# sony/DiffRoll

Hardware: AMD Instinct MI355X
Metric: piano-roll frames/sec (200-step sample) (higher is better)
Workload: dtype f32

## Files before the change

diffroll_amd/csrc/device_common.h:

```cpp
#pragma once
#include "kernels.h"

#include <algorithm>
#include <cstdio>
#include <cstdlib>
#include <type_traits>

namespace dr {

typedef float f32x16 __attribute__((ext_vector_type(16)));
typedef float f32x4 __attribute__((ext_vector_type(4)));
typedef unsigned u32x4 __attribute__((ext_vector_type(4)));

#define DR_DEVINL __device__ __forceinline__

#ifndef DR_FAULT
#define DR_FAULT 0
#endif

#ifdef DR_BOUNDS
static __device__ unsigned long long g_bounds[4];
DR_DEVINL void bounds_fail(unsigned code, long a, long b) {
    if (atomicCAS(&g_bounds[0], 0ull, (unsigned long long)code) == 0ull) { g_bounds[1] = (unsigned long long)a; g_bounds[2] = (unsigned long long)b; }
    atomicAdd(&g_bounds[3], 1ull);
// ... 5 lines not shown
#define DR_CHECK_LDS(p, lo, hi, code) do { const unsigned o_ = lds_off(p); if (o_ < (unsigned)(lo) || o_ + 16u > (unsigned)(hi)) bounds_fail((code), o_, (hi)); } while (0)
static unsigned long long g_host_violations = 0;
static void host_extent(const void* p, size_t bytes, const char* what, const char* kernel) {
    if (!p || !bytes) return;
    hipDeviceptr_t base = nullptr;
    size_t size = 0;
    if (hipMemGetAddressRange(&base, &size, (hipDeviceptr_t)p) != hipSuccess) { (void)hipGetLastError(); return; }
    if ((const char*)p < (const char*)base || (const char*)p + bytes > (const char*)base + size) {
        ++g_host_violations;
        fprintf(stderr, "[DR_BOUNDS] %s: %s needs %zu bytes at +%zd of a %zu-byte allocation\n", kernel, what, bytes,
                (ssize_t)((const char*)p - (const char*)base), size);
    }
}
static void check_gemm_extents(const GemmArgs& a, int epi, int prec, const char* kernel) {
    const size_t slab = prec ? 24576 : 16384;
    const int mts = a.mt0 + a.MT;
    host_extent(a.Wp, (size_t)mts * a.kchunks * a.taps * slab, "packed weights", kernel);
    host_extent(a.bias, (size_t)mts * 128 * 4, "bias", kernel);
    if (epi == EPI_GATE) host_extent(a.bias2, (size_t)mts * 128 * 4, "bias2", kernel);
    const long nbx = a.x_bmod ? (a.NB < a.x_bmod ? a.NB : a.x_bmod) : a.NB;
    if (!prec) host_extent(a.X, (size_t)((nbx - 1) * a.x_bs + (long)(a.x_planes - 1) * a.x_ps + (long)(a.T - 1) * a.x_fs + 4) * 4, "X", kernel);
    const long nby = a.NB + (a.dual > 0 ? a.dual : 0);
    const long planes = (a.y_rows + 3) / 4;
    if (!(a.out_s3 & 1)) host_extent(a.Y, (size_t)((nby - 1) * a.y_bs + (planes - 1) * a.y_ps + (long)(a.T - 1) * a.y_fs + 4) * 4, "Y", kernel);
    if (a.Y2 && !(a.out_s3 & 2)) host_extent(a.Y2, (size_t)((nby - 1) * a.y2_bs + (planes - 1) * a.y_ps + (long)(a.T - 1) * a.y_fs + 4) * 4, "Y2", kernel);
    const long c_hi = a.c_b0 + (a.n_cond > 1 ? a.n_cond - 1 : 0), c_last = (a.c_n > 0 && c_hi >= a.c_n) ? a.c_n - 1 : c_hi;
    if (epi == EPI_GATE && a.cond) host_extent(a.cond, (size_t)(c_last * a.c_bs + (long)mts * 128 * a.T) * 4, "conditioner", kernel);
    if (epi == EPI_GATE && a.cond2) host_extent(a.cond2, (size_t)mts * 128 * a.T * 4, "conditioner (shared)", kernel);
    if (epi == EPI_RES_SKIP && a.skip && mts * 128 > a.y_rows)
        host_extent(a.skip, (size_t)((long)(a.NB - 1) * a.s_bs + (long)(mts * 128 - a.y_rows) * a.T) * 4, "skip", kernel);
    if (a.ws) host_extent(a.ws, a.ws_floats * 4, "split-K workspace", kernel);
    if (a.ws_cnt) host_extent(a.ws_cnt, a.ws_cnt_n * 4, "split-K counters", kernel);
}
#define DR_BOUNDS_TU(tag)                                                                                       \
    hipError_t read_bounds_##tag(unsigned long long* out4) {                                                    \
        hipError_t e = hipMemcpyFromSymbol(out4, HIP_SYMBOL(g_bounds), 4 * sizeof(unsigned long long));         \
        if (e == hipSuccess && g_host_violations) { if (!out4[0]) out4[0] = 999; out4[3] += g_host_violations; } \
        return e;                                                                                               \
    }                                                                                                           \
    hipError_t reset_bounds_##tag() {                                                                           \
        unsigned long long z[4] = {0, 0, 0, 0};                                                                 \
        g_host_violations = 0;                                                                                  \
        return hipMemcpyToSymbol(HIP_SYMBOL(g_bounds), z, sizeof z);                                            \
    }
#define DR_CHECK_EXTENTS(a, epi, prec, kernel) check_gemm_extents((a), (epi), (prec), (kernel))
// ... 123 lines not shown
```

diffroll_amd/csrc/gemm.hip:

```cpp
#include "gemm_body.h"

namespace dr {

Tuning& tuning() { static Tuning t; return t; }
std::atomic<unsigned>& tuning_epoch() { static std::atomic<unsigned> n{0}; return n; }
PlanKnobs plan_knobs() {
    const Tuning& t = tuning();
    PlanKnobs k;
    k.tile = t.tile; k.pw = t.pw; k.pw_nw = t.pw_nw; k.pwk = t.pwk; k.ksplit_max = t.ksplit_max;
    k.ksplit_blocks = t.ksplit_blocks; k.stack3 = t.stack3; k.stack_fl = t.stack_fl;
    return k;
}

DR_BOUNDS_TU(gemm)
hipError_t read_bounds(unsigned long long* out4) {
    unsigned long long t[4];
    hipError_t e;
    out4[0] = out4[1] = out4[2] = out4[3] = 0;
    hipError_t (*readers[])(unsigned long long*) = {read_bounds_gemm, read_bounds_stack, read_bounds_tail};
    for (auto rd : readers) {
        if ((e = rd(t)) != hipSuccess) return e;
        if (!out4[0] && t[0]) { out4[0] = t[0]; out4[1] = t[1]; out4[2] = t[2]; }
        out4[3] += t[3];
    }
// ... 23 lines not shown
    }
    return o;
}

template <int NI, int KS, int EPI, int PREC, int FOLDP = (NI == 1)>
__global__ __launch_bounds__(512) void gemm_kernel(const GemmArgs a) {
    extern __shared__ __attribute__((aligned(16))) char smem[];
    const BlockTile bt = block_tile(a, a.ksplit);
    gemm_body<NI, KS, EPI, PREC, 0, FOLDP>(a, smem, bt.mt, bt.nt, bt.ks);
}

template <int NW>
__global__ __launch_bounds__(256) void pw_kernel(const GemmArgs a) {
    const int wave = __builtin_amdgcn_readfirstlane(threadIdx.x >> 6);
    const BlockTile bt = block_tile(a, 1);
    pw_body<NW, 0, 0>(a, bt.mt + a.mt0, bt.nt, wave);
}

template <int NW>
__global__ __launch_bounds__(256) void pwk_kernel(const GemmArgs a) {
    __shared__ float4 part[4][NW][4][64];
    const int wave = __builtin_amdgcn_readfirstlane(threadIdx.x >> 6);
    const int lane = threadIdx.x & 63;
    const int r = lane & 31, hi = lane >> 5;
    constexpr int BN = 32 * NW;
    const int RT = a.MT * 4;
    const int rt = blockIdx.x % RT + a.mt0 * 4, nt = blockIdx.x / RT;
    const int mt = rt >> 2, sr = rt & 3;
    const int tps = (a.T + BN - 1) / BN;
    const int b = nt / tps;
    const int t0 = (nt % tps) * BN;
    const int NS = a.kchunks, NSW = NS >> 2;
    const int s0 = wave * NSW;

    const __amdgpu_buffer_rsrc_t wr = __builtin_amdgcn_make_buffer_rsrc(
        (void*)(a.Wp + (long)mt * NS * 4096), 0, (unsigned)NS * 16384u, 0x00020000);
    const __amdgpu_buffer_rsrc_t xr = __builtin_amdgcn_make_buffer_rsrc(
        (void*)(a.X + (long)b * a.x_bs), 0, (unsigned)(a.x_planes * a.x_ps * 4), 0x00020000);
    const int wvo = (hi * 128 + sr * 32 + r) * 16;
    const int xps = (int)a.x_ps * 4;
    int xvo[NW];
#pragma unroll
    for (int ni = 0; ni < NW; ++ni) xvo[ni] = hi * xps + min(t0 + ni * 32 + r, a.T - 1) * 16;
    struct BF { float4 v[4][NW]; };
    auto load_a = [&](int slab) { return load_a4(wr, wvo, slab, NS, 140); };
    auto load_b = [&](int slab) -> BF {
        BF o;
#pragma unroll
        for (int g = 0; g < 4; ++g)
#pragma unroll
            for (int ni = 0; ni < NW; ++ni)
                o.v[g][ni] = buffer_load_f4(xr, xvo[ni], (slab * 8 + g * 2) * xps);
        return o;
    };
    const int p0 = mt * 128 + sr * 32 + 8 * wave + 4 * hi;
    const bool res_rows = p0 < a.y_rows;
    const float4 ebias = *reinterpret_cast<const float4*>(a.bias + p0);
    const float4 ed2 = *reinterpret_cast<const float4*>(a.d2 + (a.tsel ? (long)a.tsel[b] * a.d2_ts : 0) + min(p0, a.y_rows - 4));
    float4 eop[NW];
    {
        const float* base = res_rows ? a.Y + (long)b * a.y_bs + (long)(p0 >> 2) * a.y_ps
                                     : a.skip + (long)b * a.s_bs + (long)((p0 - a.y_rows) >> 2) * a.T * 4;
        const long fs = res_rows ? a.y_fs : 4;
#pragma unroll
        for (int ni = 0; ni < NW; ++ni) eop[ni] = *reinterpret_cast<const float4*>(base + (long)min(t0 + ni * 32 + r, a.T - 1) * fs);
    }

    f32x16 acc[NW];
#pragma unroll
    for (int ni = 0; ni < NW; ++ni)
#pragma unroll
        for (int e = 0; e < 16; ++e) acc[ni][e] = 0.f;
    AF4 aA = load_a(s0), aB;
    BF bA = load_b(s0), bB;
    auto mma = [&](const AF4& af, const BF& bf) {
#pragma unroll
        for (int g = 0; g < 4; ++g) {
// ... 34 lines not shown
            f4arr(part[w][ni][wave][lane], u);
#pragma unroll
            for (int e = 0; e < 4; ++e) v[e] += u[e];
        }
        if (res_rows) {
            float* dst = a.Y + (long)b * a.y_bs + (long)(p0 >> 2) * a.y_ps + (long)t * a.y_fs;
            residual_quad(v, ebias, eop[ni], o);
            *reinterpret_cast<float4*>(dst) = make_float4(o[0], o[1], o[2], o[3]);
            if (a.Y2) {
                float o2[4];
                hd_quad(o, ed2, o2);
                float* dst2 = a.Y2 + (long)b * a.y2_bs + (long)(p0 >> 2) * a.y_ps + (long)t * a.y_fs;
                *reinterpret_cast<float4*>(dst2) = make_float4(o2[0], o2[1], o2[2], o2[3]);
            }
        } else {
            float* dst = a.skip + (long)b * a.s_bs + ((long)((p0 - a.y_rows) >> 2) * a.T + t) * 4;
            skip_quad(v, ebias, eop[ni], a.skip_init, o);
            *reinterpret_cast<float4*>(dst) = make_float4(o[0], o[1], o[2], o[3]);
        }
    }
}

template <int NW>
static hipError_t launch_pwk_t(const GemmArgs& a, hipStream_t s) {
    const int BN = 32 * NW;
    const int NT = a.NB * ((a.T + BN - 1) / BN);
    DR_CHECK_EXTENTS(a, EPI_RES_SKIP, 0, "pwk_kernel");
    hipLaunchKernelGGL((pwk_kernel<NW>), dim3((unsigned)(a.MT * 4 * NT)), dim3(256), 0, s, a);
    return hipGetLastError();
}
hipError_t launch_pointwise_ksplit(const GemmArgs& a, int NW, hipStream_t s) {
// ... 179 lines not shown
```

diffroll_amd/csrc/gemm_body.h:

```cpp
#pragma once
#include "device_common.h"

namespace dr {

DR_DEVINL void residual_quad(const float (&v)[4], const float4 bias, const float4 prev, float (&o)[4]) {
    float bb[4], pv[4];
    f4arr(bias, bb); f4arr(prev, pv);
#pragma unroll
    for (int e = 0; e < 4; ++e) o[e] = div_sqrt2(pv[e] + (v[e] + bb[e]));
}
DR_DEVINL void skip_quad(const float (&v)[4], const float4 bias, const float4 prev, const bool skip_init, float (&o)[4]) {
    float bb[4], pv[4];
    f4arr(bias, bb); f4arr(prev, pv);
#pragma unroll
    for (int e = 0; e < 4; ++e) o[e] = skip_init ? v[e] + bb[e] : (v[e] + bb[e]) + pv[e];
}
DR_DEVINL long cond_row(const GemmArgs& a, const int b) {
    int r = a.c_b0 + b;
    if (a.c_n > 0 && r >= a.c_n) r %= a.c_n;
    return r;
}
DR_DEVINL void gate_quad(const float (&v0)[4], const float (&v1)[4], const float4 bias0, const float4 bias1,
                         const float4 cond0, const float4 cond1, const bool has_c, float (&o)[4]) {
    float b0[4], b1[4], c0[4], c1[4];
// ... 69 lines not shown
                const int sg = pl / 6, rem = pl - sg * 6, pce = rem >> 1, kq = rem & 1;
                const int pc = min(chunk * (4 * KS) + sg * 2 + kq, last_plane);
                src = Xg + (long)pce * a.x_piece + (long)pc * a.x_ps;
            } else {
                src = Xg + (long)min(chunk * XP + pl, last_plane) * a.x_ps;
            }
            const __amdgpu_buffer_rsrc_t rsrc = __builtin_amdgcn_make_buffer_rsrc((void*)src, 0, recs, 0x00020000);
            const int voff = (t0 - halo + f) * (int)a.x_fs * 4;
            float4* dst = Xs + (((chunk - c0) & 1) * XP + pl) * FW + seg * 64;
            if (f < FW) DR_CHECK_LDS(dst + lane, lds_off(Xs), lds_off(Xs) + 2u * XP * FW * 16u, code_x);
            if (f < FW) __builtin_amdgcn_raw_ptr_buffer_load_lds(rsrc, (lds_ptr)dst, 16, voff, 0, 0, AUX);
        }
    };
    if constexpr (RBN != 0) {
        auto plane_of = [&](int pl) -> const float* {
            const int row0 = mt * 128 + pl * 4;
            return (row0 < a.y_rows) ? a.Y + (long)b * a.y_bs + (long)(row0 >> 2) * a.y_ps
                                     : a.skip + (long)b * a.s_bs + (long)((row0 - a.y_rows) >> 2) * a.T * 4;
        };
        dma_tile<RBN, AUX>(Rs, plane_of, a.T, t0, pw, 4, lane, code_r);
    }
    issue(c0);
    for (int chunk = c0; chunk < c1; ++chunk) {
#if DR_FAULT != 1
        asm volatile("s_waitcnt vmcnt(0)" ::: "memory");
        __syncthreads();
#else
        __builtin_amdgcn_s_barrier();
#endif
        if (chunk + 1 < c1) issue(chunk + 1);
    }
}

// ... 318 lines not shown
    for (int pass = 0; pass < npass; ++pass) {
        const int be = b + pass * a.dual;
        const float* cbase = nullptr;
        if constexpr (EPI == EPI_GATE)
            cbase = (be < a.n_cond || !a.cond2) ? a.cond + (be < a.n_cond ? cond_row(a, be) : 0L) * a.c_bs : a.cond2;
        float4 ebias[4];
        float4 ed2[4];
        {
            const float* bsrc = a.bias;
            if constexpr (EPI == EPI_GATE) bsrc = (be < a.n_cond) ? a.bias : a.bias2;
    #pragma unroll
            for (int q = 0; q < 4; ++q) ebias[q] = *reinterpret_cast<const float4*>(bsrc + mt * 128 + wave * 32 + 8 * q + 4 * hi);
            if constexpr (EPI == EPI_RELU || EPI == EPI_RES_SKIP) {
    #pragma unroll
                for (int q = 0; q < 4; ++q) {
                    const int p0 = min(mt * 128 + wave * 32 + 8 * q + 4 * hi, a.y_rows - 4);
                    ed2[q] = *reinterpret_cast<const float4*>(a.d2 + (a.tsel ? (long)a.tsel[be] * a.d2_ts : 0) + p0);
                }
            }
        }
    #pragma unroll
        for (int ni = 0; ni < NW; ++ni) {
            const int t = t0 + ni * 32 + r;
            if constexpr (EPI == EPI_RES_SKIP) {
    #pragma unroll
                for (int q = 0; q < 4; ++q) {
                    DR_CHECK_LDS(Rs + (wave * 8 + 2 * q + hi) * BN + ni * 32 + r, xs1, rs1, 110);
                    eop[ni][q] = Rs[(wave * 8 + 2 * q + hi) * BN + ni * 32 + r];
                }
            }
            if constexpr (EPI == EPI_GATE) {
// ... 22 lines not shown
    #pragma unroll
                        for (int e = 0; e < 4; ++e) o[e] = v0[e] * v0[e] + v1[e] * v1[e];
                    }
                    if (a.out_s3 & 1) {
                        store_s3_quad<COH>(a.Y + (long)be * a.y_bs, o, c0, t, a.T, a.y_rows >> 3, a.wt_store);
                    } else {
                        float* dst = a.Y + (long)be * a.y_bs + (long)(c0 >> 2) * a.y_ps + (long)t * a.y_fs;
                        store_f4<COH>(dst, make_float4(o[0], o[1], o[2], o[3]), a.wt_store);
                    }
                } else {
                    const int p0 = mt * 128 + wave * 32 + rq;
                    float v[4], o[4];
    #pragma unroll
                    for (int e = 0; e < 4; ++e) v[e] = acc[ni][4 * q + e];
                    if constexpr (EPI == EPI_RES_SKIP) {
                        if (p0 < a.y_rows) {
                            float* dst = a.Y + (long)be * a.y_bs + (long)(p0 >> 2) * a.y_ps + (long)t * a.y_fs;
                            residual_quad(v, ebias[q], eop[ni][q], o);
                            *reinterpret_cast<float4*>(dst) = make_float4(o[0], o[1], o[2], o[3]);
                            if (a.Y2) store_y2<COH, 0>(a, be, o, ed2[q], p0, t);
                        } else {
                            float* dst = a.skip + (long)be * a.s_bs + ((long)((p0 - a.y_rows) >> 2) * a.T + t) * 4;
                            skip_quad(v, ebias[q], eop[ni][q], a.skip_init, o);
                            *reinterpret_cast<float4*>(dst) = make_float4(o[0], o[1], o[2], o[3]);
                        }
                    } else {
                        if (p0 >= a.y_rows) continue;
                        float bb[4];
                        f4arr(ebias[q], bb);
    #pragma unroll
                        for (int e = 0; e < 4; ++e) {
                            if constexpr (EPI == EPI_PLAIN) o[e] = a.alpha * v[e] + bb[e];
                            else if constexpr (EPI == EPI_RELU) o[e] = fmaxf(a.alpha * v[e] + bb[e], 0.f);
                            else if constexpr (EPI == EPI_SILU) { const float z = v[e] + bb[e]; o[e] = z * sigmoidf_(z); }
                            else o[e] = logf(v[e] + 1e-6f);
                        }
                        float* dst = a.Y + (long)be * a.y_bs + (long)(p0 >> 2) * a.y_ps + (long)t * a.y_fs;
// ... 9 lines not shown
    if (a.dbg && blockIdx.x == 0 && tid == 0) {
        a.dbg[0] = tick1 - tick0;
        a.dbg[1] = clock64() - tick0;
    }
}

template <int NW, int COH, int RLDS, int TBN = 32 * NW, int EPI = EPI_RES_SKIP>
DR_DEVINL void pw_body(const GemmArgs& a, const int mt, const int nt, const int wave, float4* Rs = nullptr, const int foff = 0) {
    static_assert(EPI == EPI_RES_SKIP || EPI == EPI_RELU || EPI == EPI_PLAIN, "pw_body epilogues");
    static_assert(EPI == EPI_RES_SKIP || !RLDS, "the LDS-resident tile belongs to the residual / skip epilogue");
    constexpr int BN = TBN;
    int lane = threadIdx.x & 63;
    if constexpr (COH) asm volatile("" : "+v"(lane));
    const int r = lane & 31, hi = lane >> 5;
    const long long tick0 = a.dbg ? clock64() : 0;

    const int tps = (a.T + BN - 1) / BN;
    const int b = nt / tps;
    const int t0 = (nt % tps) * BN + foff;
    const int NS = a.kchunks;

    const __amdgpu_buffer_rsrc_t wr = __builtin_amdgcn_make_buffer_rsrc(
        (void*)(a.Wp + (long)mt * NS * 4096), 0, (unsigned)NS * 16384u, 0x00020000);
    const __amdgpu_buffer_rsrc_t xr = __builtin_amdgcn_make_buffer_rsrc(
        (void*)(a.X + (long)b * a.x_bs), 0, (unsigned)(a.x_planes * a.x_ps * 4), 0x00020000);
    const int wvo = (hi * 128 + wave * 32 + r) * 16;
    const int xps = (int)a.x_ps * 4;
    int xvo[NW];
#pragma unroll
    for (int ni = 0; ni < NW; ++ni) xvo[ni] = hi * xps + min(t0 + ni * 32 + r, a.T - 1) * 16;
// ... 28 lines not shown
            const float4 af = kB ? aB.v[g] : aA.v[g];
#pragma unroll
            for (int ni = 0; ni < NW; ++ni) acc[ni] = __builtin_amdgcn_mfma_f32_32x32x2f32(af.x, (kB ? bB.v[g][ni] : bA.v[g][ni]).x, acc[ni], 0, 0, 0);
#pragma unroll
            for (int ni = 0; ni < NW; ++ni) acc[ni] = __builtin_amdgcn_mfma_f32_32x32x2f32(af.y, (kB ? bB.v[g][ni] : bA.v[g][ni]).y, acc[ni], 0, 0, 0);
#pragma unroll
            for (int ni = 0; ni < NW; ++ni) acc[ni] = __builtin_amdgcn_mfma_f32_32x32x2f32(af.z, (kB ? bB.v[g][ni] : bA.v[g][ni]).z, acc[ni], 0, 0, 0);
#pragma unroll
            for (int ni = 0; ni < NW; ++ni) acc[ni] = __builtin_amdgcn_mfma_f32_32x32x2f32(af.w, (kB ? bB.v[g][ni] : bA.v[g][ni]).w, acc[ni], 0, 0, 0);
        }
        constexpr int NLD = 4 + 4 * NW, PER = (16 * NW) / NLD;
        sgb_spread<NLD, PER>();
        sgb<0x8, 16 * NW - NLD * PER>();
    };
    const int rowb = mt * 128 + wave * 32 + 4 * hi;
    const bool res_rows = rowb < a.y_rows;
    float4 ebias[4], ed2[4], eop[RLDS ? 1 : NW][4];
    auto load_epilogue = [&]() {
#pragma unroll
        for (int q = 0; q < 4; ++q) {
            ebias[q] = *reinterpret_cast<const float4*>(a.bias + rowb + 8 * q);
            if constexpr (EPI == EPI_RES_SKIP)
                ed2[q] = *reinterpret_cast<const float4*>(a.d2 + (a.tsel ? (long)a.tsel[b] * a.d2_ts : 0) + min(rowb + 8 * q, a.y_rows - 4));
        }
        if constexpr (RLDS || EPI != EPI_RES_SKIP) return;
        const float* base = res_rows ? a.Y + (long)b * a.y_bs + (long)(rowb >> 2) * a.y_ps
                                     : a.skip + (long)b * a.s_bs + (long)((rowb - a.y_rows) >> 2) * a.T * 4;
        const long qs = res_rows ? 2 * a.y_ps : (long)2 * a.T * 4;
        const long fs = res_rows ? a.y_fs : 4;
#pragma unroll
        for (int ni = 0; ni < NW; ++ni) {
            const int tc = min(t0 + ni * 32 + r, a.T - 1);
#pragma unroll
            for (int q = 0; q < 4; ++q) eop[ni][q] = *reinterpret_cast<const float4*>(base + q * qs + tc * fs);
        }
    };
    int slab = 0;
    const int pre = max(NS - 2, 0) & ~1;
    for (; slab < pre; slab += 2) {
        step(std::false_type{}, slab);
        step(std::true_type{}, slab + 1);
        if (a.dbg && slab == 0 && blockIdx.x == 0 && threadIdx.x == 0) a.dbg[2] = clock64() - tick0;
// ... 3 lines not shown
    __builtin_amdgcn_sched_barrier(0);
    for (; slab + 2 <= NS; slab += 2) {
        step(std::false_type{}, slab);
        step(std::true_type{}, slab + 1);
    }
    if (slab < NS) step(std::false_type{}, slab);
    const long long tick1 = a.dbg ? clock64() : 0;
    if constexpr (RLDS) load_epilogue();

#pragma unroll
    for (int ni = 0; ni < NW; ++ni) {
        const int t = t0 + ni * 32 + r;
        if (t >= a.T) continue;
#pragma unroll
        for (int q = 0; q < 4; ++q) {
            const int p0 = rowb + 8 * q;
            float v[4], o[4];
#pragma unroll
            for (int e = 0; e < 4; ++e) v[e] = acc[ni][4 * q + e];
            if constexpr (EPI != EPI_RES_SKIP) {
                if (p0 >= a.y_rows) continue;
                float bb[4];
                f4arr(ebias[q], bb);
#pragma unroll
                for (int e = 0; e < 4; ++e) {
                    o[e] = a.alpha * v[e] + bb[e];
                    if constexpr (EPI == EPI_RELU) o[e] = fmaxf(o[e], 0.f);
                }
                float* dst = a.Y + (long)b * a.y_bs + (long)(p0 >> 2) * a.y_ps + (long)t * a.y_fs;
                store_f4<COH>(dst, make_float4(o[0], o[1], o[2], o[3]), a.wt_store);
                continue;
// ... 1 lines not shown
            float4* rs = nullptr;
            if constexpr (RLDS) rs = Rs + (wave * 8 + 2 * q + hi) * BN + foff + ni * 32 + r;
#ifdef DR_BOUNDS
            if constexpr (RLDS) DR_CHECK_LDS(rs, lds_off(Rs), lds_off(Rs) + 32u * BN * 16u, 121);
#endif
            float4 pv;
            if constexpr (RLDS) pv = *rs;
            else pv = eop[ni][q];
            if (res_rows) {
                float* dst = a.Y + (long)b * a.y_bs + (long)(p0 >> 2) * a.y_ps + (long)t * a.y_fs;
                residual_quad(v, ebias[q], pv, o);
                if constexpr (RLDS) *rs = make_float4(o[0], o[1], o[2], o[3]);
                else *reinterpret_cast<float4*>(dst) = make_float4(o[0], o[1], o[2], o[3]);
                if (a.Y2) store_y2<0, COH>(a, b, o, ed2[q], p0, t);
            } else {
                float* dst = a.skip + (long)b * a.s_bs + ((long)((p0 - a.y_rows) >> 2) * a.T + t) * 4;
                skip_quad(v, ebias[q], pv, a.skip_init, o);
                if constexpr (RLDS) *rs = make_float4(o[0], o[1], o[2], o[3]);
                else *reinterpret_cast<float4*>(dst) = make_float4(o[0], o[1], o[2], o[3]);
            }
        }
    }
    if (a.dbg && blockIdx.x == 0 && threadIdx.x == 0) {
        a.dbg[0] = tick1 - tick0;
        a.dbg[1] = clock64() - tick0;
    }
}

template <int NJ, int KS, int EPI>
DR_DEVINL void gemm16_body(const GemmArgs& a, char* smem, const int mt, const int nt) {
    static_assert(EPI == EPI_GATE || EPI == EPI_RES_SKIP, "16x16 variant: hot kernels only");
// ... 111 lines not shown
        }
    }

    const int rowb = mt * 128 + wave * 32 + kq * 4;
    float4 ebias[RT], ed2[RT];
    const float* cbase = nullptr;
    if constexpr (EPI == EPI_GATE)
        cbase = (b < a.n_cond || !a.cond2) ? a.cond + (b < a.n_cond ? cond_row(a, b) : 0L) * a.c_bs : a.cond2;
    {
        const float* bsrc = a.bias;
        if constexpr (EPI == EPI_GATE) bsrc = (b < a.n_cond) ? a.bias : a.bias2;
#pragma unroll
        for (int rt = 0; rt < RT; ++rt) {
            ebias[rt] = *reinterpret_cast<const float4*>(bsrc + rowb + rt * 16);
            if constexpr (EPI == EPI_RES_SKIP)
                ed2[rt] = *reinterpret_cast<const float4*>(a.d2 + (a.tsel ? (long)a.tsel[b] * a.d2_ts : 0) + min(rowb + rt * 16, a.y_rows - 4));
        }
    }
#pragma unroll
    for (int ct = 0; ct < CT; ++ct) {
        const int t = t0 + ct * 16 + li;
        if constexpr (EPI == EPI_GATE) {
            float4 cnd[RT];
            const int tc = min(t, a.T - 1);
            const float* cb = cbase + (long)tc * 4;
#pragma unroll
            for (int rt = 0; rt < RT; ++rt) cnd[rt] = *reinterpret_cast<const float4*>(cb + (long)((rowb + rt * 16) >> 2) * a.T * 4);
            if (t >= a.T) continue;
            const bool has_c = b < a.n_cond || a.cond2 != nullptr;
            {
                const int c0 = mt * 64 + wave * 16 + kq * 4;
// ... 6 lines not shown
                } else {
                    float* dst = a.Y + (long)b * a.y_bs + (long)(c0 >> 2) * a.y_ps + (long)t * a.y_fs;
                    *reinterpret_cast<float4*>(dst) = make_float4(o[0], o[1], o[2], o[3]);
                }
            }
        } else {
            float4 pv4[RT];
#pragma unroll
            for (int rt = 0; rt < RT; ++rt) {
                DR_CHECK_LDS(Rs + ((wave * 32 + rt * 16) / 4 + kq) * BN + ct * 16 + li, xs1, rs1, 145);
                pv4[rt] = Rs[((wave * 32 + rt * 16) / 4 + kq) * BN + ct * 16 + li];
            }
            if (t >= a.T) continue;
#pragma unroll
            for (int rt = 0; rt < RT; ++rt) {
                const int p0 = rowb + rt * 16;
                float v[4], o[4];
                f4arr(acc[rt][ct], v);
                if (p0 < a.y_rows) {
                    float* dst = a.Y + (long)b * a.y_bs + (long)(p0 >> 2) * a.y_ps + (long)t * a.y_fs;
                    residual_quad(v, ebias[rt], pv4[rt], o);
                    *reinterpret_cast<float4*>(dst) = make_float4(o[0], o[1], o[2], o[3]);
                    if (a.Y2) store_y2<0, 0>(a, b, o, ed2[rt], p0, t);
                } else {
                    float* dst = a.skip + (long)b * a.s_bs + ((long)((p0 - a.y_rows) >> 2) * a.T + t) * 4;
                    skip_quad(v, ebias[rt], pv4[rt], a.skip_init, o);
                    *reinterpret_cast<float4*>(dst) = make_float4(o[0], o[1], o[2], o[3]);
                }
            }
        }
    }
}

}
```

diffroll_amd/csrc/kernels.h:

```cpp
#pragma once
#include <hip/hip_runtime.h>
#include <stdint.h>

#include <atomic>

#include "launch_plan.h"

namespace dr {


struct Tuning {
    std::atomic<int> pack_threads{16};
    std::atomic<int> tile{0};
    std::atomic<int> pw{1};
    std::atomic<int> pw_nw{0};
    std::atomic<int> pwk{1};
    std::atomic<int> ksplit_max{16};
    std::atomic<long> ksplit_blocks{0};
    std::atomic<int> one_ks{0};
    std::atomic<int> stack3{1};
    std::atomic<int> stack_fl{0};
    std::atomic<int> tail_t4{0};
    std::atomic<int> xcd_n{-1};
    std::atomic<int> xcd_model{1};
// ... 5 lines not shown
PlanKnobs plan_knobs();

struct GemmArgs {
    const float* Wp;
    const float* bias;
    const float* bias2;
    const float* X;
    long x_bs, x_ps, x_fs;
    long x_piece;
    int x_planes;
    int x_bmod;
    int NB, T;
    int taps, dil;
    int kchunks;
    int MT;
    int mt0;
    float* Y;
    long y_bs, y_ps, y_fs;
    long y2_bs;
    int out_s3;
    float* Y2;
    const float* d2;
    const int* tsel;
    long d2_ts;
    int y_rows;
    const float* cond;
    long c_bs;
    int c_b0, c_n;
    const float* cond2;
    int n_cond;
    int dual;
    float* skip;
    long s_bs;
    int skip_init;
    float alpha;
    int xcd_n;
    float* ws;
    unsigned* ws_cnt;
    size_t ws_floats, ws_cnt_n;
    int ksplit;
    long long* dbg;
    int lds_bytes;
    int fold128;
    int nofold64;
    int wt_store;
};

hipError_t init_kernels();
hipError_t read_bounds(unsigned long long* out4);
// ... 128 lines not shown
```

diffroll_amd/csrc/launch_plan.h:

```cpp
#pragma once
#include <algorithm>
#include <cstddef>

#include "../../include/diffroll_amd.h"

namespace dr {

enum Epilogue : int {
    EPI_PLAIN = 0,
    EPI_RELU = 1,
    EPI_SILU = 2,
    EPI_GATE = 3,
    EPI_RES_SKIP = 4,
    EPI_POWER = 5,
    EPI_LOG = 6
};

constexpr int DR_STACK_MAX_LAYERS = 30;
constexpr int STACK_GROUPS = 512;
constexpr size_t SK_WS_FLOATS = (size_t)16 << 20, SK_CNT_N = 4096;

struct PlanKnobs {
    int tile = 0, pw = 1, pw_nw = 0, pwk = 1, ksplit_max = 16;
    long ksplit_blocks = 0;
    int stack3 = 1, stack_fl = 0;
};

inline int gemm_block_frames(int NI) { return (NI == 3 || NI == 5) ? 32 * NI : 64 * NI; }
inline size_t gemm_lds_bytes(int NI, int KS, int taps, int dil, int prec, int epi) {
    const int halo = ((taps - 1) / 2) * dil;
    const int BN = gemm_block_frames(NI);
// ... 194 lines not shown
```

diffroll_amd/csrc/pack.hip:

```cpp
#include "engine_state.h"

#include <mutex>

namespace drh {

template <class F>
int parallel_for(dr_engine* e, int n, F fn) {
    const int cap = tuning().pack_threads;
    const int hw = (int)std::thread::hardware_concurrency();
    const int nt = std::max(1, std::min(std::min(n, cap), hw > 0 ? hw : 1));
    std::atomic<bool> failed{false};
    auto guarded = [&](int i) {
        try { fn(i); } catch (...) { failed.store(true); }
    };
    if (nt == 1) {
        for (int i = 0; i < n && !failed.load(); ++i) guarded(i);
    } else {
        std::atomic<int> next{0};
        std::vector<std::thread> th;
        try {
            for (int t = 0; t < nt; ++t)
                th.emplace_back([&]() { for (int i = next.fetch_add(1); i < n && !failed.load(); i = next.fetch_add(1)) guarded(i); });
        } catch (...) { failed.store(true); }
        for (auto& t : th) t.join();
// ... 174 lines not shown

int ensure_s3(dr_engine* e) {
    if (e->s3_ready || !e->committed) return DR_OK;
    const int C = e->C, Cp = e->Cp, L = e->L, K = e->K;
    std::vector<std::vector<uint16_t>> c3(L), o3(L);
    int prc = parallel_for(e, L, [&](int l) {
        const std::string pre = "residual_layers." + std::to_string(l) + ".";
        const auto& Wd = *find_param(e, pre + "dilated_conv.weight");
        const auto& Wo = *find_param(e, pre + "output_projection.weight");
        const int MTc = Cp / 64;
        c3[l] = pack_weights_s3(MTc, Cp / 32, K, [&](int pr, int ch, int j) {
            int mi, c; paired_row(pr, mi, c);
            return (c < C && ch < C) ? Wd[((size_t)(mi * C + c) * C + ch) * K + j] : 0.f;
        });
        o3[l] = pack_weights_s3(MTc, Cp / 32, 1, [&](int pr, int ch, int) {
            const int half = pr >= Cp, c = pr - half * Cp;
            return (c < C && ch < C) ? Wo[(size_t)(half * C + c) * C + ch] : 0.f;
        });
    });
    if (prc) return prc;
    for (int l = 0; l < L; ++l) {
        int rc;
        if ((rc = upload_bytes(e, c3[l].data(), c3[l].size() * 2, &e->layers[l].conv_w3)) ||
            (rc = upload_bytes(e, o3[l].data(), o3[l].size() * 2, &e->layers[l].out_w3)))
            return rc;
        c3[l] = {}; o3[l] = {};
    }
    { StagerLock sl; HIPCHK(e, sl.s->drain()); }
    e->s3_ready = true;
    return DR_OK;
}
// ... 56 lines not shown
        });
        k.bconv.assign(MTc * 128, 0.f); k.bconv_u.assign(MTc * 128, 0.f); k.bconv_z.assign(MTc * 128, 0.f); k.bcond.assign(MTc * 128, 0.f);
        for (int pr = 0; pr < MTc * 128; ++pr) {
            int mi, c; paired_row(pr, mi, c);
            if (c >= C) continue;
            const int o = mi * C + c;
            double sw = 0.0;
            for (int m = 0; m < NM; ++m) sw += (double)Wc[(size_t)o * NM + m];
            const float cu = (float)((double)Bc[o] - sw);
            k.bconv[pr] = Bd[o];
            k.bconv_u[pr] = Bd[o] + cu;
            k.bconv_z[pr] = Bd[o] + Bc[o];
            k.bcond[pr] = Bc[o];
        }
        k.pout = pack_weights(MTc, Cp / 32, 1, [&](int pr, int ch, int) {
            const int half = pr >= Cp, c = pr - half * Cp;
            return (c < C && ch < C) ? Wo[(size_t)(half * C + c) * C + ch] : 0.f;
        });
        k.bout.assign(MTc * 128, 0.f);
        for (int pr = 0; pr < 2 * Cp; ++pr) {
            const int half = pr >= Cp, c = pr - half * Cp;
            if (c < C) k.bout[pr] = Bo[half * C + c];
        }
    });
    if (rc) return rc;
    e->t_pack_s = now_s() - tp0;
    const double tu0 = now_s();
    for (int l = 0; l < L; ++l) {
        LayerW& lw = e->layers[l];
        lw.dil = 1;
        for (int q = 0; q < l % e->cfg.dilation_bound; ++q) lw.dil *= e->cfg.dilation_base;
        LayerPack& k = packs[l];
        if ((rc = upload(e, k.pconv, &lw.conv_w)) || (rc = upload(e, k.bconv, &lw.conv_b)) ||
            (rc = upload(e, k.bconv_u, &lw.conv_b_u)) || (rc = upload(e, k.bconv_z, &lw.conv_b_z)) ||
            (rc = upload(e, k.pcond, &lw.cond_w)) ||
            (rc = upload(e, k.bcond, &lw.cond_b)) || (rc = upload(e, k.pout, &lw.out_w)) ||
// ... 140 lines not shown
```

diffroll_amd/csrc/plan.hip:

```cpp
#include "engine_state.h"

namespace drh {

hipError_t launch_tiled(const GemmArgs& a, int epi, Tile t, hipStream_t s, int prec) {
    if (t.flavor == 3) return launch_pointwise_ksplit(a, t.n, s);
    if (t.flavor == 2) return launch_pointwise(a, t.n, s);
    return t.flavor == 1 ? launch_gemm16(a, epi, t.n, s) : launch_gemm(a, epi, t.n, s, prec);
}
void allow_splitk(const dr_engine* e, GemmArgs& a) {
    a.ws = e->sk_ws; a.ws_cnt = e->sk_cnt;
    a.ws_floats = SK_WS_FLOATS; a.ws_cnt_n = SK_CNT_N;
}

const float* g_zero_vecs[MAX_DEVICES] = {};
const float* zero_vec() {
    int dev = 0;
    (void)hipGetDevice(&dev);
    return (dev >= 0 && dev < MAX_DEVICES) ? g_zero_vecs[dev] : nullptr;
}

GemmArgs p4_gemm(const float* Wp, const float* bias, int MT, const float* X, int planes, int NB, int T) {
    GemmArgs a{};
    a.d2 = zero_vec();
    a.Wp = Wp; a.bias = bias ? bias : zero_vec(); a.MT = MT;
// ... 193 lines not shown
    const long act_bs = (long)Cp * T;
    const LayerW& w = e->layers[l];
    GemmArgs a = p4_gemm(prec ? w.out_w3 : w.out_w, w.out_b, Cp / 64, e->g, Cp / 4, NB, T);
    if (prec) s3_in(a, e->g3, Cp, T);
    p4_out(a, e->h, Cp / 4, T, Cp);
    if (l + 1 < L) {
        a.d2 = e->d_dtab + ((v.tsel ? 0 : (size_t)v.t * L) + l + 1) * Cp;
        a.tsel = v.tsel; a.d2_ts = (long)L * Cp;
        if (prec) { a.Y2 = e->hd3; a.y2_bs = act_bs + act_bs / 2; a.out_s3 = 2; }
        else { a.Y2 = e->hd; a.y2_bs = act_bs; }
    }
    a.skip = e->skip; a.s_bs = (long)Cp * T; a.skip_init = (l == 0);
    allow_splitk(e, a);
    if (e->stack_dbg_on && l + 2 == L) a.dbg = e->stack_dbg + 96;
    Tile tile = pick_pointwise_tile(k, Cp / 64, NB, T, prec);
    if (l + 1 == L && tile.flavor >= 2) {
        const int first = Cp / 128, count = Cp / 64 - first;
        const Tile half = pick_pointwise_tile(k, count, NB, T, prec, Cp / 32);
        if (half.flavor == tile.flavor) { tile = half; a.MT = count; a.mt0 = first; }
    }
    HIPCHK(e, launch_tiled(a, EPI_RES_SKIP, tile, v.st, prec));
    return DR_OK;
}

static int launch_tail_step(const Eval& v, const NetPlan& p, const PlanKnobs& k, TailPlan* tail) {
    dr_engine* e = v.e;
    const int Cp = e->Cp, L = e->L, T = v.T;
    NetPlan np{};
    bool prime = false;
    if (tail->next_t >= 0) {
        np = plan_network(NetShape{tail->next.NB, tail->next.n_cond, v.bmod, T, Cp, L, e->K, e->max_dil, e->prec, e->n_cus,
                                   e->fused.active(), e->opt_blocked, e->opt_tail, false, true}, k);
        prime = np.use_tail;
    }
    TailArgs ta{};
// ... 157 lines not shown
```

diffroll_amd/csrc/stack.hip:

```cpp
#include "gemm_body.h"
#include "persistent.h"

namespace dr {

DR_BOUNDS_TU(stack)

template <int FL, int FOLDP = 1, int PREC = 0>
__global__ __launch_bounds__(512) void stack_kernel(const StackArgs s_by_value) {
    extern __shared__ __attribute__((aligned(16))) char smem[];
    (void)s_by_value;
    typedef const __attribute__((address_space(4))) StackArgs* KernArgs;
    const KernArgs sp = (KernArgs)__builtin_amdgcn_kernarg_segment_ptr();
    const __attribute__((address_space(4))) StackArgs& s = *sp;
    static_assert(FL == 1 || FL == 2 || (FL == 5 && FOLDP == 1 && PREC == 0), "block flavours");
    constexpr int BN = FL == 5 ? 160 : 64 * FL;
    constexpr int RP = 32;
    constexpr int RWL = (BN + 63) / 64;
    const int wave = __builtin_amdgcn_readfirstlane(threadIdx.x >> 6);
    const int MT = s.Cp >> 6;
    const int MB = MT;
    const int tps = (s.T + BN - 1) / BN;
    const unsigned gsize = (unsigned)(MB * tps);
    int mt, nt, grp, member;
    if (s.xcd_n) {
// ... 4 lines not shown
        member = blockIdx.x % (int)gsize;
        grp = blockIdx.x / (int)gsize;
    }
    if (grp >= s.NB) return;
    mt = member % MB;
    nt = grp * tps + member / MB;
    const unsigned pending_timeout = __hip_atomic_load(s.derr, __ATOMIC_RELAXED, __HIP_MEMORY_SCOPE_AGENT);
    DR_CHECK(grp >= 0 && grp < 512 && (long)grp * gsize + member < 1024, 130, grp, member);
    unsigned* ctr = s.bar + 4 * grp;
    const long act_bs = (long)s.Cp * s.T;
    const int P = s.Cp >> 2;
    unsigned episode = 0;
    float4* Rs = reinterpret_cast<float4*>(smem + s.rs_off);
    const int b_ = nt / tps, t0_ = (nt % tps) * BN;
    auto tile_plane = [&](int pl, bool& is_res) -> float* {
        const int row0 = mt * 128 + pl * 4;
        is_res = row0 < s.Cp;
        return is_res ? s.h + (long)b_ * act_bs + (long)(row0 >> 2) * s.T * 4
                      : s.skip + (long)b_ * act_bs + (long)((row0 - s.Cp) >> 2) * s.T * 4;
    };
    if constexpr (PREC) {
        if (pending_timeout) return;
    } else {
#ifdef DR_BOUNDS
        if (threadIdx.x == 0) DR_CHECK(s.rs_off + RP * BN * 16 + 16 <= s.lds_bytes && lds_off(smem) == 0u, 132, s.rs_off, s.lds_bytes);
#endif
        dma_tile<BN, 0>(Rs, [&](int pl) { bool is_res; return tile_plane(pl, is_res); }, s.T, t0_, wave, 8, threadIdx.x & 63, 131);
        if (pending_timeout) return;
        if (s.p0 & 1) {
            asm volatile("s_waitcnt vmcnt(0)" ::: "memory");
            __syncthreads();
        }
    }
    int wt_store = 1;
// ... 30 lines not shown
                a.taps = s.taps; a.dil = ly.dil;
                a.cond = ly.cond; a.cond2 = ly.cond2; a.c_bs = s.c_bs; a.c_b0 = s.c_b0; a.c_n = s.c_n; a.n_cond = s.n_cond;
                a.Y = s.g; a.y_bs = s3_bs; a.out_s3 = 1;
                gemm_body<FL, 1, EPI_GATE, 1, 1, FOLDP>(a, smem, mt, nt, 0);
            } else {
                a.Wp = ly.out_w; a.bias = ly.out_b;
                a.X = s.g; a.x_bs = s3_bs; a.x_piece = (long)(s.Cp >> 3) * s.T * 4; a.x_planes = s.Cp >> 3;
                a.taps = 1; a.dil = 1;
                a.Y = s.h;
                const bool last = (l + 1 == s.L);
                if (!last) {
                    a.Y2 = s.hd; a.y2_bs = s3_bs; a.out_s3 = 2;
                    a.d2 = s.d2 + (long)(l + 1) * s.Cp; a.tsel = s.tsel; a.d2_ts = s.d2_ts;
                }
                a.skip = s.skip; a.s_bs = act_bs; a.skip_init = (l == 0);
                const bool idle = last && mt < (s.Cp >> 7);
                const int tps64 = (s.T + 63) >> 6;
                const int b_ = nt / tps, ti = nt % tps;
#pragma unroll 1
                for (int half = 0; half < BN / 64; ++half) {
                    const int t64 = ti * (BN / 64) + half;
                    if (half) {
                        asm volatile("s_waitcnt vmcnt(0)" ::: "memory");
                        __syncthreads();
                    }
                    if (!idle && t64 < tps64) gemm_body<1, 4, EPI_RES_SKIP, 1, 1>(a, smem, mt, b_ * tps64 + t64, 0);
                }
            }
        } else
        if ((p & 1) == 0) {
            a.Wp = ly.conv_w; a.bias = ly.conv_b; a.bias2 = ly.conv_b2;
            a.X = s.hd; a.taps = s.taps; a.dil = ly.dil;
            a.cond = ly.cond; a.cond2 = ly.cond2; a.c_bs = s.c_bs; a.c_b0 = s.c_b0; a.c_n = s.c_n; a.n_cond = s.n_cond;
            a.Y = s.g;
            if (s.dbg && p + 2 >= s.p1) a.dbg = s.dbg + 64;
            gemm_body<FL, 1, EPI_GATE, 0, 1, FOLDP>(a, smem, mt, nt, 0);
            if (wave == 4) __builtin_amdgcn_fence(__ATOMIC_ACQUIRE, "agent");
            if (wave >= 4 && s.warm) {
                const int be = nt / tps;
                if (be < s.n_cond)
                    l2_touch(ly.cond + cond_row(a, be) * s.c_bs + (long)mt * 32 * s.T * 4, (unsigned)(32 * s.T * 16), wave - 4, 4);
                l2_touch(ly.out_w + (long)mt * (s.Cp >> 5) * 4096, (unsigned)((s.Cp >> 5) * 16384), wave - 4, 4);
            }
        } else {
            a.Wp = ly.out_w; a.bias = ly.out_b;
            a.X = s.g; a.taps = 1; a.dil = 1;
            a.Y = s.h;
            const bool last = (l + 1 == s.L);
            if (!last) {
                a.Y2 = s.hd; a.y2_bs = act_bs;
                a.d2 = s.d2 + (long)(l + 1) * s.Cp; a.tsel = s.tsel; a.d2_ts = s.d2_ts;
            }
            a.skip = s.skip; a.s_bs = act_bs; a.skip_init = (l == 0);
            const bool idle = last && mt < (s.Cp >> 7);
            if (s.dbg && p + 3 == s.p1) a.dbg = s.dbg + 96;
            if constexpr (FL == 2) {
                if (!idle) pw_body<2, 1, 1, 128>(a, mt, nt, wave & 3, Rs, (wave >> 2) * 64);
            } else if constexpr (FL == 5) {
                if (!idle) {
                    if (wave < 4) pw_body<3, 1, 1, 160>(a, mt, nt, wave, Rs, 0);
                    else pw_body<2, 1, 1, 160>(a, mt, nt, wave - 4, Rs, 96);
                }
            } else {
                if (wave < 4 && !idle) pw_body<BN / 32, 1, 1>(a, mt, nt, wave, Rs);
            }
            if (wave >= 4 && s.warm && !last) {
                const __attribute__((address_space(4))) StackLayer& nx = sp->layer[l + 1];
                l2_touch(nx.conv_w + (long)mt * (s.Cp >> 5) * s.taps * 4096, (unsigned)(2 * s.taps * 16384), wave - 4, 4);
            }
        }
        if (p + 1 < s.p1) {
            group_barrier<false>(ctr, ++episode * (gsize + DR_FAULT_EXTRA(s)), s.err, s.derr);
            if (episode == 1) {
                if (threadIdx.x == 0) {
                    unsigned same = 1;
                    for (unsigned i = 0; i < gsize; ++i)
                        same &= (__hip_atomic_load(s.xid + (long)grp * gsize + i, __ATOMIC_RELAXED, __HIP_MEMORY_SCOPE_AGENT) == my_tag);
                    same_xcd_s = same;
                }
// ... 82 lines not shown
```

Baseline: 2257.

## Interleave residual and skip output rows per 128-row weight tile

Repacks the output-projection weights so each 128-row M tile holds 64 residual rows and 64 skip rows, instead of all residual rows first and then all skip rows. On the last layer, where only skip rows are needed, every tile now does half its work and waves whose rows are residual exit early. Before, the first half of the tiles sat idle and the rest did full work. This spreads the last-layer work evenly across blocks and drops the mt0 offset, but the half-wave early exits add branching and may leave occupancy uneven within a block.

```diff
diff --git a/diffroll_amd/csrc/device_common.h b/diffroll_amd/csrc/device_common.h
--- a/diffroll_amd/csrc/device_common.h
+++ b/diffroll_amd/csrc/device_common.h
@@ -43,7 +43,7 @@
 }
 static void check_gemm_extents(const GemmArgs& a, int epi, int prec, const char* kernel) {
     const size_t slab = prec ? 24576 : 16384;
-    const int mts = a.mt0 + a.MT;
+    const int mts = a.MT;
     host_extent(a.Wp, (size_t)mts * a.kchunks * a.taps * slab, "packed weights", kernel);
     host_extent(a.bias, (size_t)mts * 128 * 4, "bias", kernel);
     if (epi == EPI_GATE) host_extent(a.bias2, (size_t)mts * 128 * 4, "bias2", kernel);
@@ -56,8 +56,8 @@
     const long c_hi = a.c_b0 + (a.n_cond > 1 ? a.n_cond - 1 : 0), c_last = (a.c_n > 0 && c_hi >= a.c_n) ? a.c_n - 1 : c_hi;
     if (epi == EPI_GATE && a.cond) host_extent(a.cond, (size_t)(c_last * a.c_bs + (long)mts * 128 * a.T) * 4, "conditioner", kernel);
     if (epi == EPI_GATE && a.cond2) host_extent(a.cond2, (size_t)mts * 128 * a.T * 4, "conditioner (shared)", kernel);
-    if (epi == EPI_RES_SKIP && a.skip && mts * 128 > a.y_rows)
-        host_extent(a.skip, (size_t)((long)(a.NB - 1) * a.s_bs + (long)(mts * 128 - a.y_rows) * a.T) * 4, "skip", kernel);
+    if (epi == EPI_RES_SKIP && a.skip)
+        host_extent(a.skip, (size_t)((long)(a.NB - 1) * a.s_bs + (long)mts * 64 * a.T) * 4, "skip", kernel);
     if (a.ws) host_extent(a.ws, a.ws_floats * 4, "split-K workspace", kernel);
     if (a.ws_cnt) host_extent(a.ws_cnt, a.ws_cnt_n * 4, "split-K counters", kernel);
 }
diff --git a/diffroll_amd/csrc/gemm.hip b/diffroll_amd/csrc/gemm.hip
--- a/diffroll_amd/csrc/gemm.hip
+++ b/diffroll_amd/csrc/gemm.hip
@@ -61,7 +61,7 @@
 __global__ __launch_bounds__(256) void pw_kernel(const GemmArgs a) {
     const int wave = __builtin_amdgcn_readfirstlane(threadIdx.x >> 6);
     const BlockTile bt = block_tile(a, 1);
-    pw_body<NW, 0, 0>(a, bt.mt + a.mt0, bt.nt, wave);
+    pw_body<NW, 0, 0>(a, bt.mt, bt.nt, wave);
 }
 
 template <int NW>
@@ -72,8 +72,9 @@
     const int r = lane & 31, hi = lane >> 5;
     constexpr int BN = 32 * NW;
     const int RT = a.MT * 4;
-    const int rt = blockIdx.x % RT + a.mt0 * 4, nt = blockIdx.x / RT;
+    const int rt = blockIdx.x % RT, nt = blockIdx.x / RT;
     const int mt = rt >> 2, sr = rt & 3;
+    if (a.skip_only && !res_skip_half(sr * 32)) return;
     const int tps = (a.T + BN - 1) / BN;
     const int b = nt / tps;
     const int t0 = (nt % tps) * BN;
@@ -100,14 +101,15 @@
                 o.v[g][ni] = buffer_load_f4(xr, xvo[ni], (slab * 8 + g * 2) * xps);
         return o;
     };
-    const int p0 = mt * 128 + sr * 32 + 8 * wave + 4 * hi;
-    const bool res_rows = p0 < a.y_rows;
-    const float4 ebias = *reinterpret_cast<const float4*>(a.bias + p0);
-    const float4 ed2 = *reinterpret_cast<const float4*>(a.d2 + (a.tsel ? (long)a.tsel[b] * a.d2_ts : 0) + min(p0, a.y_rows - 4));
+    const int pr = mt * 128 + sr * 32 + 8 * wave + 4 * hi;
+    const bool res_rows = !res_skip_half(pr);
+    const int p0 = res_skip_channel(pr);
+    const float4 ebias = *reinterpret_cast<const float4*>(a.bias + pr);
+    const float4 ed2 = *reinterpret_cast<const float4*>(a.d2 + (a.tsel ? (long)a.tsel[b] * a.d2_ts : 0) + p0);
     float4 eop[NW];
     {
         const float* base = res_rows ? a.Y + (long)b * a.y_bs + (long)(p0 >> 2) * a.y_ps
-                                     : a.skip + (long)b * a.s_bs + (long)((p0 - a.y_rows) >> 2) * a.T * 4;
+                                     : a.skip + (long)b * a.s_bs + (long)(p0 >> 2) * a.T * 4;
         const long fs = res_rows ? a.y_fs : 4;
 #pragma unroll
         for (int ni = 0; ni < NW; ++ni) eop[ni] = *reinterpret_cast<const float4*>(base + (long)min(t0 + ni * 32 + r, a.T - 1) * fs);
@@ -172,7 +174,7 @@
                 *reinterpret_cast<float4*>(dst2) = make_float4(o2[0], o2[1], o2[2], o2[3]);
             }
         } else {
-            float* dst = a.skip + (long)b * a.s_bs + ((long)((p0 - a.y_rows) >> 2) * a.T + t) * 4;
+            float* dst = a.skip + (long)b * a.s_bs + ((long)(p0 >> 2) * a.T + t) * 4;
             skip_quad(v, ebias, eop[ni], a.skip_init, o);
             *reinterpret_cast<float4*>(dst) = make_float4(o[0], o[1], o[2], o[3]);
         }
diff --git a/diffroll_amd/csrc/gemm_body.h b/diffroll_amd/csrc/gemm_body.h
--- a/diffroll_amd/csrc/gemm_body.h
+++ b/diffroll_amd/csrc/gemm_body.h
@@ -107,9 +107,9 @@
     };
     if constexpr (RBN != 0) {
         auto plane_of = [&](int pl) -> const float* {
-            const int row0 = mt * 128 + pl * 4;
-            return (row0 < a.y_rows) ? a.Y + (long)b * a.y_bs + (long)(row0 >> 2) * a.y_ps
-                                     : a.skip + (long)b * a.s_bs + (long)((row0 - a.y_rows) >> 2) * a.T * 4;
+            const int cpl = mt * 16 + (pl & 15);
+            return (pl < 16) ? a.Y + (long)b * a.y_bs + (long)cpl * a.y_ps
+                             : a.skip + (long)b * a.s_bs + (long)cpl * a.T * 4;
         };
         dma_tile<RBN, AUX>(Rs, plane_of, a.T, t0, pw, 4, lane, code_r);
     }
@@ -458,7 +458,8 @@
             if constexpr (EPI == EPI_RELU || EPI == EPI_RES_SKIP) {
     #pragma unroll
                 for (int q = 0; q < 4; ++q) {
-                    const int p0 = min(mt * 128 + wave * 32 + 8 * q + 4 * hi, a.y_rows - 4);
+                    const int pr = mt * 128 + wave * 32 + 8 * q + 4 * hi;
+                    const int p0 = EPI == EPI_RES_SKIP ? res_skip_channel(pr) : min(pr, a.y_rows - 4);
                     ed2[q] = *reinterpret_cast<const float4*>(a.d2 + (a.tsel ? (long)a.tsel[be] * a.d2_ts : 0) + p0);
                 }
             }
@@ -511,13 +512,14 @@
     #pragma unroll
                     for (int e = 0; e < 4; ++e) v[e] = acc[ni][4 * q + e];
                     if constexpr (EPI == EPI_RES_SKIP) {
-                        if (p0 < a.y_rows) {
-                            float* dst = a.Y + (long)be * a.y_bs + (long)(p0 >> 2) * a.y_ps + (long)t * a.y_fs;
+                        const int c0 = res_skip_channel(p0);
+                        if (!res_skip_half(p0)) {
+                            float* dst = a.Y + (long)be * a.y_bs + (long)(c0 >> 2) * a.y_ps + (long)t * a.y_fs;
                             residual_quad(v, ebias[q], eop[ni][q], o);
                             *reinterpret_cast<float4*>(dst) = make_float4(o[0], o[1], o[2], o[3]);
-                            if (a.Y2) store_y2<COH, 0>(a, be, o, ed2[q], p0, t);
+                            if (a.Y2) store_y2<COH, 0>(a, be, o, ed2[q], c0, t);
                         } else {
-                            float* dst = a.skip + (long)be * a.s_bs + ((long)((p0 - a.y_rows) >> 2) * a.T + t) * 4;
+                            float* dst = a.skip + (long)be * a.s_bs + ((long)(c0 >> 2) * a.T + t) * 4;
                             skip_quad(v, ebias[q], eop[ni][q], a.skip_init, o);
                             *reinterpret_cast<float4*>(dst) = make_float4(o[0], o[1], o[2], o[3]);
                         }
@@ -557,6 +559,9 @@
     if constexpr (COH) asm volatile("" : "+v"(lane));
     const int r = lane & 31, hi = lane >> 5;
     const long long tick0 = a.dbg ? clock64() : 0;
+    if constexpr (EPI == EPI_RES_SKIP) {
+        if (a.skip_only && !res_skip_half(wave * 32)) return;
+    }
 
     const int tps = (a.T + BN - 1) / BN;
     const int b = nt / tps;
@@ -615,18 +620,19 @@
         sgb<0x8, 16 * NW - NLD * PER>();
     };
     const int rowb = mt * 128 + wave * 32 + 4 * hi;
-    const bool res_rows = rowb < a.y_rows;
+    const bool res_rows = EPI != EPI_RES_SKIP || !res_skip_half(rowb);
+    const int chb = EPI == EPI_RES_SKIP ? res_skip_channel(rowb) : rowb;
     float4 ebias[4], ed2[4], eop[RLDS ? 1 : NW][4];
     auto load_epilogue = [&]() {
 #pragma unroll
         for (int q = 0; q < 4; ++q) {
             ebias[q] = *reinterpret_cast<const float4*>(a.bias + rowb + 8 * q);
             if constexpr (EPI == EPI_RES_SKIP)
-                ed2[q] = *reinterpret_cast<const float4*>(a.d2 + (a.tsel ? (long)a.tsel[b] * a.d2_ts : 0) + min(rowb + 8 * q, a.y_rows - 4));
+                ed2[q] = *reinterpret_cast<const float4*>(a.d2 + (a.tsel ? (long)a.tsel[b] * a.d2_ts : 0) + chb + 8 * q);
         }
         if constexpr (RLDS || EPI != EPI_RES_SKIP) return;
-        const float* base = res_rows ? a.Y + (long)b * a.y_bs + (long)(rowb >> 2) * a.y_ps
-                                     : a.skip + (long)b * a.s_bs + (long)((rowb - a.y_rows) >> 2) * a.T * 4;
+        const float* base = res_rows ? a.Y + (long)b * a.y_bs + (long)(chb >> 2) * a.y_ps
+                                     : a.skip + (long)b * a.s_bs + (long)(chb >> 2) * a.T * 4;
         const long qs = res_rows ? 2 * a.y_ps : (long)2 * a.T * 4;
         const long fs = res_rows ? a.y_fs : 4;
 #pragma unroll
@@ -660,7 +666,7 @@
         if (t >= a.T) continue;
 #pragma unroll
         for (int q = 0; q < 4; ++q) {
-            const int p0 = rowb + 8 * q;
+            const int p0 = chb + 8 * q;
             float v[4], o[4];
 #pragma unroll
             for (int e = 0; e < 4; ++e) v[e] = acc[ni][4 * q + e];
@@ -692,7 +698,7 @@
                 else *reinterpret_cast<float4*>(dst) = make_float4(o[0], o[1], o[2], o[3]);
                 if (a.Y2) store_y2<0, COH>(a, b, o, ed2[q], p0, t);
             } else {
-                float* dst = a.skip + (long)b * a.s_bs + ((long)((p0 - a.y_rows) >> 2) * a.T + t) * 4;
+                float* dst = a.skip + (long)b * a.s_bs + ((long)(p0 >> 2) * a.T + t) * 4;
                 skip_quad(v, ebias[q], pv, a.skip_init, o);
                 if constexpr (RLDS) *rs = make_float4(o[0], o[1], o[2], o[3]);
                 else *reinterpret_cast<float4*>(dst) = make_float4(o[0], o[1], o[2], o[3]);
@@ -834,7 +840,7 @@
         for (int rt = 0; rt < RT; ++rt) {
             ebias[rt] = *reinterpret_cast<const float4*>(bsrc + rowb + rt * 16);
             if constexpr (EPI == EPI_RES_SKIP)
-                ed2[rt] = *reinterpret_cast<const float4*>(a.d2 + (a.tsel ? (long)a.tsel[b] * a.d2_ts : 0) + min(rowb + rt * 16, a.y_rows - 4));
+                ed2[rt] = *reinterpret_cast<const float4*>(a.d2 + (a.tsel ? (long)a.tsel[b] * a.d2_ts : 0) + res_skip_channel(rowb + rt * 16));
         }
     }
 #pragma unroll
@@ -871,16 +877,16 @@
             if (t >= a.T) continue;
 #pragma unroll
             for (int rt = 0; rt < RT; ++rt) {
-                const int p0 = rowb + rt * 16;
+                const int p0 = res_skip_channel(rowb + rt * 16);
                 float v[4], o[4];
                 f4arr(acc[rt][ct], v);
-                if (p0 < a.y_rows) {
+                if (!res_skip_half(rowb)) {
                     float* dst = a.Y + (long)b * a.y_bs + (long)(p0 >> 2) * a.y_ps + (long)t * a.y_fs;
                     residual_quad(v, ebias[rt], pv4[rt], o);
                     *reinterpret_cast<float4*>(dst) = make_float4(o[0], o[1], o[2], o[3]);
                     if (a.Y2) store_y2<0, 0>(a, b, o, ed2[rt], p0, t);
                 } else {
-                    float* dst = a.skip + (long)b * a.s_bs + ((long)((p0 - a.y_rows) >> 2) * a.T + t) * 4;
+                    float* dst = a.skip + (long)b * a.s_bs + ((long)(p0 >> 2) * a.T + t) * 4;
                     skip_quad(v, ebias[rt], pv4[rt], a.skip_init, o);
                     *reinterpret_cast<float4*>(dst) = make_float4(o[0], o[1], o[2], o[3]);
                 }
diff --git a/diffroll_amd/csrc/kernels.h b/diffroll_amd/csrc/kernels.h
--- a/diffroll_amd/csrc/kernels.h
+++ b/diffroll_amd/csrc/kernels.h
@@ -43,7 +43,6 @@
     int taps, dil;
     int kchunks;
     int MT;
-    int mt0;
     float* Y;
     long y_bs, y_ps, y_fs;
     long y2_bs;
@@ -62,6 +61,7 @@
     float* skip;
     long s_bs;
     int skip_init;
+    int skip_only;
     float alpha;
     int xcd_n;
     float* ws;
diff --git a/diffroll_amd/csrc/launch_plan.h b/diffroll_amd/csrc/launch_plan.h
--- a/diffroll_amd/csrc/launch_plan.h
+++ b/diffroll_amd/csrc/launch_plan.h
@@ -15,6 +15,9 @@
     EPI_POWER = 5,
     EPI_LOG = 6
 };
+
+constexpr int res_skip_half(int prow) { return (prow >> 6) & 1; }
+constexpr int res_skip_channel(int prow) { return (prow >> 7) * 64 + (prow & 63); }
 
 constexpr int DR_STACK_MAX_LAYERS = 30;
 constexpr int STACK_GROUPS = 512;
diff --git a/diffroll_amd/csrc/pack.hip b/diffroll_amd/csrc/pack.hip
--- a/diffroll_amd/csrc/pack.hip
+++ b/diffroll_amd/csrc/pack.hip
@@ -212,7 +212,7 @@
             return (c < C && ch < C) ? Wd[((size_t)(mi * C + c) * C + ch) * K + j] : 0.f;
         });
         o3[l] = pack_weights_s3(MTc, Cp / 32, 1, [&](int pr, int ch, int) {
-            const int half = pr >= Cp, c = pr - half * Cp;
+            const int half = dr::res_skip_half(pr), c = dr::res_skip_channel(pr);
             return (c < C && ch < C) ? Wo[(size_t)(half * C + c) * C + ch] : 0.f;
         });
     });
@@ -299,12 +299,12 @@
             k.bcond[pr] = Bc[o];
         }
         k.pout = pack_weights(MTc, Cp / 32, 1, [&](int pr, int ch, int) {
-            const int half = pr >= Cp, c = pr - half * Cp;
+            const int half = dr::res_skip_half(pr), c = dr::res_skip_channel(pr);
             return (c < C && ch < C) ? Wo[(size_t)(half * C + c) * C + ch] : 0.f;
         });
         k.bout.assign(MTc * 128, 0.f);
         for (int pr = 0; pr < 2 * Cp; ++pr) {
-            const int half = pr >= Cp, c = pr - half * Cp;
+            const int half = dr::res_skip_half(pr), c = dr::res_skip_channel(pr);
             if (c < C) k.bout[pr] = Bo[half * C + c];
         }
     });
diff --git a/diffroll_amd/csrc/plan.hip b/diffroll_amd/csrc/plan.hip
--- a/diffroll_amd/csrc/plan.hip
+++ b/diffroll_amd/csrc/plan.hip
@@ -231,11 +231,7 @@
     allow_splitk(e, a);
     if (e->stack_dbg_on && l + 2 == L) a.dbg = e->stack_dbg + 96;
     Tile tile = pick_pointwise_tile(k, Cp / 64, NB, T, prec);
-    if (l + 1 == L && tile.flavor >= 2) {
-        const int first = Cp / 128, count = Cp / 64 - first;
-        const Tile half = pick_pointwise_tile(k, count, NB, T, prec, Cp / 32);
-        if (half.flavor == tile.flavor) { tile = half; a.MT = count; a.mt0 = first; }
-    }
+    if (l + 1 == L && tile.flavor >= 2) a.skip_only = 1;
     HIPCHK(e, launch_tiled(a, EPI_RES_SKIP, tile, v.st, prec));
     return DR_OK;
 }
diff --git a/diffroll_amd/csrc/stack.hip b/diffroll_amd/csrc/stack.hip
--- a/diffroll_amd/csrc/stack.hip
+++ b/diffroll_amd/csrc/stack.hip
@@ -42,10 +42,8 @@
     float4* Rs = reinterpret_cast<float4*>(smem + s.rs_off);
     const int b_ = nt / tps, t0_ = (nt % tps) * BN;
     auto tile_plane = [&](int pl, bool& is_res) -> float* {
-        const int row0 = mt * 128 + pl * 4;
-        is_res = row0 < s.Cp;
-        return is_res ? s.h + (long)b_ * act_bs + (long)(row0 >> 2) * s.T * 4
-                      : s.skip + (long)b_ * act_bs + (long)((row0 - s.Cp) >> 2) * s.T * 4;
+        is_res = pl < 16;
+        return (is_res ? s.h : s.skip) + (long)b_ * act_bs + (long)(mt * 16 + (pl & 15)) * s.T * 4;
     };
     if constexpr (PREC) {
         if (pending_timeout) return;
@@ -106,7 +104,6 @@
                     a.d2 = s.d2 + (long)(l + 1) * s.Cp; a.tsel = s.tsel; a.d2_ts = s.d2_ts;
                 }
                 a.skip = s.skip; a.s_bs = act_bs; a.skip_init = (l == 0);
-                const bool idle = last && mt < (s.Cp >> 7);
                 const int tps64 = (s.T + 63) >> 6;
                 const int b_ = nt / tps, ti = nt % tps;
 #pragma unroll 1
@@ -116,7 +113,7 @@
                         asm volatile("s_waitcnt vmcnt(0)" ::: "memory");
                         __syncthreads();
                     }
-                    if (!idle && t64 < tps64) gemm_body<1, 4, EPI_RES_SKIP, 1, 1>(a, smem, mt, b_ * tps64 + t64, 0);
+                    if (t64 < tps64) gemm_body<1, 4, EPI_RES_SKIP, 1, 1>(a, smem, mt, b_ * tps64 + t64, 0);
                 }
             }
         } else
@@ -144,17 +141,15 @@
                 a.d2 = s.d2 + (long)(l + 1) * s.Cp; a.tsel = s.tsel; a.d2_ts = s.d2_ts;
             }
             a.skip = s.skip; a.s_bs = act_bs; a.skip_init = (l == 0);
-            const bool idle = last && mt < (s.Cp >> 7);
+            a.skip_only = last;
             if (s.dbg && p + 3 == s.p1) a.dbg = s.dbg + 96;
             if constexpr (FL == 2) {
-                if (!idle) pw_body<2, 1, 1, 128>(a, mt, nt, wave & 3, Rs, (wave >> 2) * 64);
+                pw_body<2, 1, 1, 128>(a, mt, nt, wave & 3, Rs, (wave >> 2) * 64);
             } else if constexpr (FL == 5) {
-                if (!idle) {
-                    if (wave < 4) pw_body<3, 1, 1, 160>(a, mt, nt, wave, Rs, 0);
-                    else pw_body<2, 1, 1, 160>(a, mt, nt, wave - 4, Rs, 96);
-                }
+                if (wave < 4) pw_body<3, 1, 1, 160>(a, mt, nt, wave, Rs, 0);
+                else pw_body<2, 1, 1, 160>(a, mt, nt, wave - 4, Rs, 96);
             } else {
-                if (wave < 4 && !idle) pw_body<BN / 32, 1, 1>(a, mt, nt, wave, Rs);
+                if (wave < 4) pw_body<BN / 32, 1, 1>(a, mt, nt, wave, Rs);
             }
             if (wave >= 4 && s.warm && !last) {
                 const __attribute__((address_space(4))) StackLayer& nx = sp->layer[l + 1];
```

New measurement: 2259, median of 5. Within noise of the previous version (+0.1%).
